# qinjr/SCoRe

Measured on AMD Instinct MI355X. Metric: train samples/sec @ batch=1024, higher is better.
Workload: dtype f32

## Files before the change

include/score_hip.h:

```cpp
#ifndef SCORE_HIP_H
#define SCORE_HIP_H

#include <stdint.h>

#ifdef __cplusplus
extern "C" {
#endif

#define SCORE_E_BADARG   (-1)
#define SCORE_E_SHAPE    (-2)
#define SCORE_E_WORKSPACE (-3)
#define SCORE_E_INDEX    (-4)

typedef void* score_context_t;
int score_context_create(score_context_t* ctx);
int score_context_destroy(score_context_t ctx);
int score_event_create(void** event);
int score_event_destroy(void* event);
int score_event_record(void* event, void* stream);
int score_stream_wait_event(void* stream, void* event);
int score_event_query(void* event);
int score_event_synchronize(void* event);

typedef struct {
// ... 178 lines not shown
  int32_t gemm_mode;
  int32_t debug_flags;
  uint8_t* row_flags;
  void* gather_done_event;
  void* plan_done_event;
  const score_step_scalars_t* step_scalars;
  score_context_t context;
  int32_t* id_status;
  void* grads_done_event;
  void* loss_done_event;
  float* loss_host;
  float* plan_workspace;
  const uint8_t* drop_mask2;
} score_state_t;

int score_id_status(int32_t* id_status, int32_t* bits, int32_t clear, void* stream);

int score_gemm_forms(const score_config_t* cfg, const score_state_t* st, int32_t B, int32_t active_slices,
                     int32_t* x_form, int32_t* dx_form);

int score_persample_form(const score_config_t* cfg, const score_state_t* st, int32_t B, int32_t active_slices);

int score_index_plan(const score_config_t* cfg, const score_state_t* st, const score_batch_t* batch,
                     int32_t n_shards, int32_t dedup, void* stream);

int score_sort_pairs(uint32_t* keys, uint32_t* vals, uint32_t* keys_alt, uint32_t* vals_alt, int64_t n, int32_t key_bits,
                     void* temp, int64_t temp_bytes, int32_t* result_in_alt, void* stream);
int64_t score_sort_pairs_temp_bytes(int64_t n);

int score_segment_sum_rows(const int32_t* rows, const float* src, int64_t n, int32_t D, int64_t n_out_rows,
                           float* out, uint8_t* row_flags, void* scratch, int64_t scratch_bytes, void* stream);
int64_t score_segment_sum_scratch_bytes(int64_t n, int32_t D);

int score_rows_accumulate(const int32_t* rows, const float* src, int64_t n, int32_t D, int64_t n_out_rows,
                          float* out, uint8_t* row_flags, void* stream);
int score_rows_accumulate_multi(const int32_t* rows, const float* src, const int64_t* offsets, int32_t n_sources, int32_t D,
                                int64_t n_out_rows, float* out, uint8_t* row_flags, void* stream);

int score_forward(const score_config_t* cfg, const score_state_t* st, const score_batch_t* batch,
                  float reg_lambda, float keep_prob, const uint8_t* drop_mask0,
                  const uint8_t* drop_mask1, uint64_t drop_seed, void* const* stage_events,
                  void* stream);

int score_backward(const score_config_t* cfg, const score_state_t* st, const score_batch_t* batch,
                   float keep_prob, float* grad_w, float* grad_table, void* const* stage_events,
                   void* stream);

typedef struct {
  const int32_t* user_seq;
  const int32_t* length;
  const int32_t* target_user;
  const int32_t* cand_items;
  const int32_t* label;
  int32_t L, C;
  int32_t active_slices;
} score_rank_batch_t;

int score_rank_workspace_bytes(const score_config_t* cfg, int32_t L, int32_t C, int64_t* bytes);
int score_rank_forward(const score_config_t* cfg, const score_state_t* st, const score_rank_batch_t* rb,
                       float reg_lambda, float* y_pred , float* loss , void* stream);

#define SCORE_CATALOG_KMAX 128
typedef struct {
  const int32_t* item_rows;
  int32_t N;
  float* zcat;
// ... 269 lines not shown
```

score_amd/_lib.py:

```python
import ctypes as C
import os

_HERE = os.path.dirname(os.path.abspath(__file__))
LIB_PATH = os.path.join(_HERE, "lib", "libscore_hip.so")

MODEL_TYPES = {"SCORE": 0, "RIA": 1, "RCA": 2, "SCORE_USER": 3, "SCORE_ITEM": 4, "RRN": 5, "GCMC": 6, "GRU4Rec": 7, "Caser": 8, "DELF": 9,
               "DEEMS": 10, "SVDpp": 11, "SASRec": 12}

MAX_PARAM_ENTRIES = 48

c_f = C.c_void_p
c_i = C.c_void_p


class Config(C.Structure):
    _fields_ = [("feature_size", C.c_int64), ("eb_dim", C.c_int32), ("hidden_size", C.c_int32),
                ("max_time_len", C.c_int32), ("obj_per_time_slice", C.c_int32),
                ("user_fnum", C.c_int32), ("item_fnum", C.c_int32), ("model_type", C.c_int32)]


class ParamEntry(C.Structure):
    _fields_ = [("name", C.c_char * 64), ("offset", C.c_int64), ("rows", C.c_int32), ("cols", C.c_int32),
                ("regularised", C.c_int32), ("init", C.c_int32)]

# ... 203 lines not shown
    "score_gemm_panel_images": [C.c_int32, C.c_int32, C.c_int32, C.c_int32, C.c_void_p, C.c_int32, c_f, C.c_int64, C.c_void_p],
    "score_gemm_panel_run": [C.c_int32, C.c_int32, C.c_int32, C.c_int32, C.c_void_p, C.c_int32, C.c_void_p, C.c_int32, C.c_void_p,
                             c_f, C.c_int64, C.c_void_p],
    "score_gemm_panel_products": [C.c_int32, C.c_int32, C.c_int32, C.c_int32, C.c_int32, C.c_void_p, C.c_int32, C.c_void_p,
                                  C.c_int32, C.c_void_p, C.c_int32, C.c_void_p, c_f, C.c_int64, C.c_void_p],
    "score_gru_fwd": [C.c_int32, C.c_int32, C.c_int32, c_f, c_f, C.c_int32, c_f, C.c_int32, c_i, c_f, C.c_int32,
                      c_f, c_f, C.c_void_p],
    "score_gru_bwd": [C.c_int32, C.c_int32, C.c_int32, c_f, C.c_int32, c_f, C.c_int32, c_i, c_f, C.c_int32, c_f,
                      c_f, C.c_int32, c_f, c_f, c_f, c_f, C.c_void_p],
    "score_adam": [c_f, c_f, c_f, c_f, C.c_int64, C.c_int64, C.c_float, C.c_float, C.c_float, C.c_float,
                   C.c_float, C.POINTER(Guard), C.c_void_p],
    "score_adam_dev": [c_f, c_f, c_f, c_f, C.c_int64, C.c_int64, C.c_float, C.c_void_p, C.c_float, C.c_float, C.c_float,
                       C.POINTER(Guard), C.c_void_p],
    "score_adam_rows_dev": [c_f, c_f, c_f, c_f, C.c_int64, C.c_int32, C.c_void_p, C.c_void_p, C.c_float, C.c_float,
                            C.c_float, C.POINTER(Guard), C.c_void_p],
    "score_adam_rows": [c_f, c_f, c_f, c_f, C.c_int64, C.c_int32, C.c_void_p, C.c_float, C.c_float, C.c_float,
                        C.c_float, C.POINTER(Guard), C.c_void_p],
    "score_adam_rows_and_dense": [c_f, c_f, c_f, c_f, C.c_int64, C.c_int32, C.c_void_p, c_f, c_f, c_f, c_f, C.c_int64, C.c_int64,
                                  C.c_float, C.c_float, C.c_float, C.c_float, C.c_float, C.POINTER(Guard), C.c_void_p],
    "score_adam_touched": [C.POINTER(AdamTable), C.c_uint32, C.c_float, C.c_void_p],
    "score_adam_touched_and_dense": [C.POINTER(AdamTable), C.c_uint32, C.c_float, c_f, c_f, c_f, c_f, C.c_int64, C.c_int64,
                                     C.c_float, C.c_void_p, C.c_void_p],
    "score_adam_unmark": [C.POINTER(AdamTable), C.c_uint32, C.c_void_p],
    "score_adam_catchup_ids": [C.POINTER(AdamTable), c_i, C.c_int64, C.c_uint32, C.c_void_p],
    "score_adam_catchup_ids_through": [C.POINTER(AdamTable), c_i, C.c_int64, C.c_uint32, C.c_float, C.c_void_p],
    "score_adam_catchup_rows": [C.POINTER(AdamTable), C.c_int64, C.c_int64, C.c_uint32, C.c_void_p],
    "score_index_plan": [C.POINTER(Config), C.POINTER(State), C.POINTER(Batch), C.c_int32, C.c_int32, C.c_void_p],
    "score_sort_pairs": [C.c_void_p, C.c_void_p, C.c_void_p, C.c_void_p, C.c_int64, C.c_int32, C.c_void_p, C.c_int64,
                         C.POINTER(C.c_int32), C.c_void_p],
    "score_sort_pairs_temp_bytes": [C.c_int64],
    "score_segment_sum_rows": [c_i, c_f, C.c_int64, C.c_int32, C.c_int64, c_f, C.c_void_p, C.c_void_p, C.c_int64,
                               C.c_void_p],
    "score_segment_sum_scratch_bytes": [C.c_int64, C.c_int32],
    "score_rows_accumulate": [c_i, c_f, C.c_int64, C.c_int32, C.c_int64, c_f, C.c_void_p, C.c_void_p],
    "score_rows_accumulate_multi": [c_i, c_f, C.POINTER(C.c_int64), C.c_int32, C.c_int32, C.c_int64, c_f, C.c_void_p, C.c_void_p],
    "score_auc_logloss": [c_f, c_i, C.c_int64, C.c_void_p, C.c_void_p, C.c_int64, C.c_void_p],
    "score_auc_scratch_bytes": [C.c_int64],
    "score_ranking_quality": [c_f, c_i, C.c_int64, C.c_int32, c_f, c_i, c_f, C.c_int64, C.c_void_p],
    "score_persample_form": [C.POINTER(Config), C.POINTER(State), C.c_int32, C.c_int32],
    "score_event_create": [C.POINTER(C.c_void_p)],
    "score_event_destroy": [C.c_void_p],
    "score_event_record": [C.c_void_p, C.c_void_p],
    "score_stream_wait_event": [C.c_void_p, C.c_void_p],
    "score_event_query": [C.c_void_p],
    "score_event_synchronize": [C.c_void_p],
    "score_abi_struct_sizes": [C.POINTER(C.c_int64), C.c_int32],
    "score_train_step": [C.POINTER(Config), C.POINTER(State), C.POINTER(Batch), C.POINTER(TrainStep), C.c_void_p],
    "score_gemm_forms": [C.POINTER(Config), C.POINTER(State), C.c_int32, C.c_int32, C.POINTER(C.c_int32), C.POINTER(C.c_int32)],
    "score_forward": [C.POINTER(Config), C.POINTER(State), C.POINTER(Batch), C.c_float, C.c_float, C.c_void_p,
                      C.c_void_p, C.c_uint64, C.POINTER(C.c_void_p), C.c_void_p],
    "score_backward": [C.POINTER(Config), C.POINTER(State), C.POINTER(Batch), C.c_float, c_f, c_f,
                       C.POINTER(C.c_void_p), C.c_void_p],
    "score_rank_workspace_bytes": [C.POINTER(Config), C.c_int32, C.c_int32, C.POINTER(C.c_int64)],
    "score_rank_forward": [C.POINTER(Config), C.POINTER(State), C.POINTER(RankBatch), C.c_float, c_f, c_f, C.c_void_p],
    "score_catalog_build": [C.POINTER(Config), C.POINTER(State), C.POINTER(Catalog), C.c_void_p],
    "score_catalog_plan": [C.POINTER(Config), C.c_int32, C.c_int32, C.c_int32, C.POINTER(C.c_int32), C.POINTER(C.c_int32),
                           C.POINTER(C.c_int64)],
    "score_catalog_topk": [C.POINTER(Config), C.POINTER(State), C.POINTER(Catalog), C.POINTER(CatalogLines), C.c_int32, c_i, c_f, c_f,
                           C.c_void_p],
    "score_catalog_struct_sizes": [C.POINTER(C.c_int64), C.c_int32],
    "score_catalog_cands_plan": [C.POINTER(Config), C.c_int32, C.c_int32, C.c_int32, C.POINTER(C.c_int32), C.POINTER(C.c_int32),
                                 C.POINTER(C.c_int64)],
    "score_catalog_topk_in": [C.POINTER(Config), C.POINTER(State), C.POINTER(Catalog), C.POINTER(CatalogLines),
                              C.POINTER(CatalogCands), C.c_int32, c_i, c_f, c_f, C.c_void_p],
    "score_catalog_cands_struct_sizes": [C.POINTER(C.c_int64), C.c_int32],
    "score_catalog_ranks_plan": [C.POINTER(Config), C.c_int32, C.c_int32, C.POINTER(C.c_int32), C.POINTER(C.c_int32),
# ... 190 lines not shown
```

score_amd/csrc/engine.hip:

```cpp
#include <string.h>
#include <stdlib.h>
#include <stdio.h>
#include <math.h>
#include <mutex>
#include <new>
#include "common.h"
#include "kernels.h"
#include "persample.h"

namespace {

const int FC1 = 200, FC2 = 80, AT1 = 80, AT2 = 40;
const int CASER_L = SCORE_CASER_L, CASER_HPAD = SCORE_CASER_HPAD;
const int MAX_ENTRIES = 48;

enum Family { FAM_SLICE, FAM_GCMC, FAM_G4R, FAM_CASER, FAM_DELF, FAM_DEEMS, FAM_SVDPP, FAM_SASREC };

struct Dims {
  int64_t N;
  int D, H, T, K, Fu, Fi, mt;
  int Du, Di, I, Dq, NI, Dk, Dhead, nstate;
  int Is[2];
  bool coattn, attn;
  Family family;
// ... 489 lines not shown
  hipStream_t st; hipEvent_t a, b, c;
  hipError_t e = hipStreamCreateWithFlags(&st, hipStreamNonBlocking);
  if (e != hipSuccess) return (int)e;
  if ((e = hipEventCreateWithFlags(&a, SCORE_DEVICE_EVENT_FLAGS)) != hipSuccess) { hipStreamDestroy(st); return (int)e; }
  if ((e = hipEventCreateWithFlags(&b, SCORE_DEVICE_EVENT_FLAGS)) != hipSuccess) { hipEventDestroy(a); hipStreamDestroy(st); return (int)e; }
  if ((e = hipEventCreateWithFlags(&c, SCORE_DEVICE_EVENT_FLAGS)) != hipSuccess) { hipEventDestroy(a); hipEventDestroy(b); hipStreamDestroy(st); return (int)e; }
  sd->st = st; sd->fork = a; sd->join = b; sd->wx = c; sd->device = dev; sd->fwd_on = nullptr;
  return 0;
}
static void side_stream_release(SideStream* sd) {
  if (!sd->st) return;
  hipStreamSynchronize(sd->st);
  hipEventDestroy(sd->fork); hipEventDestroy(sd->join); hipEventDestroy(sd->wx);
  hipStreamDestroy(sd->st);
  sd->st = nullptr;
}
#define SCORE_MAX_DEVICES 16
static SideStream g_default_ctx[SCORE_MAX_DEVICES];
static std::mutex g_default_mu;
static int side_stream(const score_state_t* st, SideStream** out) {
  if (st && st->context) { *out = reinterpret_cast<SideStream*>(st->context); return 0; }
  int dev = 0;
  if (hipGetDevice(&dev) != hipSuccess || dev < 0 || dev >= SCORE_MAX_DEVICES) return SCORE_E_BADARG;
  std::lock_guard<std::mutex> lock(g_default_mu);
  SideStream& sd = g_default_ctx[dev];
  if (!sd.st) SCORE_TRY(side_stream_create(&sd));
  *out = &sd;
  return 0;
}
enum {
  DF_GRU_STEPWISE = 1, DF_HEAD_FUSED_ANY_B = 2, DF_GRU_F32_REC = 4, DF_NO_PANEL = 8, DF_PANEL_DX = 16, DF_SORT_LIB = 32,
  DF_HEAD_UNFUSED = 64, DF_ATTN_UNFUSED = 128, DF_SORT_OWN = 256, DF_NO_PS = 512, DF_PS_FWD_ONLY = 1024, DF_PS_BWD_ONLY = 2048,
  DF_ONE_STREAM = 4096, DF_G4R_COMPOSED = 8192, DF_COATTN_ALL_ROWS = 32768,
  DF_COATTN_META_AHEAD = 65536, DF_COATTN_FWD_ONE_UNIT = 131072
};
static inline int coattn_fwd_ch_of(const score_state_t* st) { return (st->debug_flags >> 20) & 15; }
struct Flags {
  bool gru_stepwise, head_fused_any_b, gru_f32_rec, no_panel, panel_dx, sort_lib, head_unfused, attn_unfused, sort_own, no_ps,
      ps_fwd_only, ps_bwd_only, one_stream, g4r_composed, coattn_all_rows, coattn_meta_ahead, coattn_fwd_one_unit;
};
static inline Flags flags_of(const score_state_t* st) {
  auto on = [st](int bit) { return (st->debug_flags & bit) != 0; };
  Flags o;
  o.gru_stepwise = on(DF_GRU_STEPWISE); o.head_fused_any_b = on(DF_HEAD_FUSED_ANY_B); o.gru_f32_rec = on(DF_GRU_F32_REC);
  o.no_panel = on(DF_NO_PANEL); o.panel_dx = on(DF_PANEL_DX); o.sort_lib = on(DF_SORT_LIB); o.sort_own = on(DF_SORT_OWN);
  o.head_unfused = on(DF_HEAD_UNFUSED); o.attn_unfused = on(DF_ATTN_UNFUSED); o.no_ps = on(DF_NO_PS);
  o.ps_fwd_only = on(DF_PS_FWD_ONLY); o.ps_bwd_only = on(DF_PS_BWD_ONLY); o.one_stream = on(DF_ONE_STREAM);
  o.g4r_composed = on(DF_G4R_COMPOSED); o.coattn_all_rows = on(DF_COATTN_ALL_ROWS);
  o.coattn_meta_ahead = on(DF_COATTN_META_AHEAD); o.coattn_fwd_one_unit = on(DF_COATTN_FWD_ONE_UNIT);
  return o;
}
static int side_stream(const score_state_t* st, hipStream_t s, SideStream** out) {
  SideStream* real = nullptr;
  SCORE_TRY(side_stream(st, &real));
  if (!st || !flags_of(st).one_stream) { *out = real; return 0; }
  static thread_local SideStream inl;
  const hipStream_t was = inl.fwd_on;
  inl = *real; inl.st = s; inl.fwd_on = was;
  *out = &inl;
  return 0;
}
static inline int fork_side(SideStream* side, hipStream_t s) {
  HIPTRY(hipEventRecord(side->fork, s));
  HIPTRY(hipStreamWaitEvent(side->st, side->fork, 0));
  return 0;
}

#define G(call) SCORE_TRY(call)
static inline int gemm_mode_call(int x3, int tr, int M, int N, int K, const float* A, int lda, const float* B,
                                 int ldb, float* C, int ldc, const float* bias, int flags, float keep,
                                 const uint8_t* mask, uint64_t seed, float* scratch, int64_t scratch_floats,
                                 void* s) {
  return score_gemm(tr, M, N, K, A, lda, B, ldb, C, ldc, bias, flags | x3, keep, mask, seed, scratch, scratch_floats,
                    s);
}
#define EV(i) \
  do { if (stage_events && stage_events[i]) HIPTRY(hipEventRecord((hipEvent_t)stage_events[i], s)); } while (0)

static inline uint32_t clamp_rows(int64_t n) { return (uint32_t)(n < 0x80000000ll ? n : 0x80000000ll); }
static inline int global_batch(const score_state_t* st, int B) { return st->global_batch > 0 ? st->global_batch : B; }

struct Pass {
// ... 295 lines not shown
    pg.A = A ? A[side] : nullptr; pg.img = p->img[g]; pg.C = C ? C[side] + half * p->Nh : nullptr;
    pg.bias = which == 0 ? cat + (int64_t)d.Is[side] * 3 * H + half * p->Nh : nullptr;
  }
}
static int panel_prep(const Pass& c, int which, hipStream_t on) {
  PanelGroups p;
  panel_groups(c, which, nullptr, nullptr, &p);
  return score_gemm_panel_prep(p.n, p.src, 3 * c.H, p.trans, p.Nh, p.K, p.img, on);
}
static int panel_launch(const Pass& c, int which, const float* const* A, float* const* C) {
  PanelGroups p;
  panel_groups(c, which, A, C, &p);
  return score_gemm_panel(p.n, p.pg, c.BT, p.Nh, p.K, p.lda, p.ldc, c.s);
}

static int loss_tail_at(const Pass& c, SideStream* sd, float reg_lambda, int n, const float* lossb, float* loss, int Bg) {
  hipStream_t ls = c.s;
  if (c.st->loss_done_event) { G(fork_side(sd, c.s)); ls = sd->st; }
  G(score_launch_loss_final(n, lossb, loss, reg_lambda, c.ws + c.w.part, Bg, ls, c.st->id_status));
  if (c.st->loss_done_event) HIPTRY(hipEventRecord((hipEvent_t)c.st->loss_done_event, ls));
  return 0;
}
static int loss_tail(const Pass& c, SideStream* sd, float reg_lambda) {
  return loss_tail_at(c, sd, reg_lambda, c.B, c.ws + c.w.lossb, c.ws + c.w.loss, c.Bg);
}

static int row_scatter(const Pass& c, float* plan, float* grad_table) {
  const Dims& d = c.d; const Params& P = c.P; const WS& w = c.w; float* ws = c.ws; const float* W = c.W;
  PullArgs pa;
  memset(&pa, 0, sizeof(pa));
  pa.D = d.D; pa.K = d.K; pa.zero_is_dummy = 1;
  pa.flags = c.st->scatter_mode == 0 ? c.st->row_flags : nullptr;
  pa.uid = c.st->scatter_mode == 2 ? reinterpret_cast<const uint32_t*>(ws + w.uid) : nullptr;
  const float invK = 1.0f / (float)d.K;
  const float* Gm[6] = {ws + w.dxside[0], ws + w.dxside[1], ws + w.dxside[0], ws + w.dxside[1], ws + w.dtgt, ws + w.dtgt};
  const int ldg[6] = {d.I, d.I, d.I, d.I, d.Dq, d.Dq};
  const int gcol[6] = {0, d.Du, d.Di, 0, 0, d.Du};
  for (int g = 0; g < 6; ++g) { pa.G[g] = Gm[g]; pa.ldg[g] = ldg[g]; pa.gcol[g] = gcol[g]; pa.constA[g] = 1.0f; }
  if (d.coattn) {
    pa.cA[0] = ws + w.pcoef[0]; pa.cA[2] = ws + w.pcoef[1];
    pa.constA[1] = invK; pa.constA[3] = invK;
    pa.cB[0] = pa.cB[1] = ws + w.dzcoef[0]; pa.cB[2] = pa.cB[3] = ws + w.dzcoef[1];
    pa.Wv[0] = W + P.ca_w[0] + d.Di; pa.Wv[1] = W + P.ca_w[0] + 2 * d.Di;
    pa.Wv[2] = W + P.ca_w[1] + d.Du; pa.Wv[3] = W + P.ca_w[1] + 2 * d.Du;
  }
  const int64_t n_occ = (int64_t)c.B * (2 * (int64_t)c.T * d.K * (d.Fu + d.Fi) + d.Fu + d.Fi);
  return score_launch_pull(pa, reinterpret_cast<uint32_t*>(plan + w.keys_out), reinterpret_cast<uint32_t*>(plan + w.vals_out),
                           n_occ + 1, grad_table, ws + w.partials, w.partial_floats, c.s);
}

struct GradQueues { GemmQueue gq; ColsumJobs cq; };
static inline void queues_init(GradQueues* q) { q->gq.n = 0; q->cq.n = 0; q->cq.part_used = 0; }
static int queue_head(const Pass& c, GradQueues* q, float* gw, bool bn1_sums) {
  const Dims& d = c.d; const Params& P = c.P; const WS& w = c.w; float* ws = c.ws; const int B = c.B;
  G(gemm_queue_add(&q->gq, FC2, 1, B, ws + w.f2, FC2, ws + w.dlogit, 1, gw + P.fc_w[2], 1));
  G(colsum_queue_add(&q->cq, ws + w.dlogit, B, 1, 1, gw + P.fc_b[2], 0));
  G(gemm_queue_add(&q->gq, FC1, FC2, B, ws + w.f1, FC1, ws + w.dz2, FC2, gw + P.fc_w[1], FC2));
  G(colsum_queue_add(&q->cq, ws + w.dz2, B, FC2, FC2, gw + P.fc_b[1], 0));
  G(gemm_queue_add(&q->gq, d.Dhead, FC1, B, ws + w.bn, d.Dhead, ws + w.dz1, FC1, gw + P.fc_w[0], FC1));
  G(colsum_queue_add(&q->cq, ws + w.dz1, B, FC1, FC1, gw + P.fc_b[0], 0));
  if (bn1_sums) {
    G(colsum_queue_add(&q->cq, ws + w.dgstage, B, d.Dhead, d.Dhead, gw + P.bn_g, 0));
    G(colsum_queue_add(&q->cq, ws + w.dbn, B, d.Dhead, d.Dhead, gw + P.bn_b, 0));
  }
  return 0;
}
// ... 1546 lines not shown
```

score_amd/csrc/kernels.h:

```cpp
#pragma once
#include "common.h"

#define GEMM_GROUP_MAX 16
struct GemmProb {
  const float* A; const float* B; float* C; float* slab;
  const float* bias;
  int M, N, K, lda, ldb, ldc, k_chunk, gx, gy, nblocks;
};
struct GemmGroup { int n; int total_blocks; GemmProb p[GEMM_GROUP_MAX]; };
enum { GF_BIAS = 1, GF_RELU = 2, GF_ACC = 4, GF_DROP = 8, GF_X3 = 16, GF_X3F = 32, GF_RELUGRAD = 64 };
__device__ __forceinline__ int64_t bias_index(int flags, int row, int col, int N) {
  const int g = flags >> 16;
  return g ? (int64_t)(row / g) * N + col : col;
}
__device__ __forceinline__ float gemm_epilogue(float v, int row, int col, int N, const float* bias, int flags,
                                               float keep, const uint8_t* mask, uint64_t seed) {
  if (flags & GF_BIAS) v += bias[bias_index(flags, row, col, N)];
  if (flags & GF_RELU) v = fmaxf(v, 0.f);
  if (flags & GF_DROP) {
    uint64_t e = (uint64_t)row * (uint64_t)N + (uint64_t)col;
    bool on = mask ? (mask[e] != 0) : (hash_uniform(seed, e) < keep);
    v = on ? v / keep : 0.f;
  }
  if (flags & GF_RELUGRAD) {
// ... 112 lines not shown
                                float* logit, float* y, float* lossb, float* dlogit, int Bglobal, hipStream_t s,
                                const uint64_t* seed_dev = nullptr, float* dz2 = nullptr, int single_launch = 0);
bool score_head_fwd_fused_fits(int B, int Dh, int N1, int N2);
int score_launch_head_bwd_fused(int B, int Dh, int N1, int N2, const float* dz2, const float* W2, const float* f1, float keep,
                                const float* W1, const float* x, const float* gamma, float rs, float* dz1, float* dbn,
                                float* dhead, float* tmp, hipStream_t s);
int score_launch_attn_fwd_fused(int B, int T, int H, int NI, int N1, int N2, const float* q, const float* ur,
                                const float* ir, const float* info, const float* Weff, const float* qz, const float* W4,
                                const float* b4, const float* w5, const float* b5, const int32_t* length, float* inp,
                                float* a1, float* a2, float* score, float* head, int ldh, int off_u, int off_i,
                                hipStream_t s, int weff_copies = 1, int64_t weff_copy_stride = 0);
int score_launch_outer_relu_bwd(int B, int NF, const float* dlogit, const float* w, const float* f, float keep,
                                float* dz, hipStream_t s);
int score_launch_copy2d(int64_t rows, int cols, const float* src, int lds_, float* dst, int ldd, hipStream_t s);

struct PlanFillArgs {
  const int32_t* idx[6];
  int64_t off[7];
  int F[6];
  int K, G, shift;
  int T, TA;
  uint32_t n_rows;
  int32_t* id_status;
};
struct PullArgs {
  const float* G[6]; int ldg[6]; int gcol[6];
  const float* cA[6]; const float* cB[6];
  const float* Wv[6];
  float constA[6];
  const uint32_t* uid;
  int D, K, LPRp;
  int zero_is_dummy;
  uint8_t* flags;
};
struct PlanRemapArgs { int32_t* out[6]; int F[6]; int K; int T, TA; };
int score_launch_plan_unique(const PlanRemapArgs& ra, const uint32_t* keys, const uint32_t* vals, int64_t n,
                             uint32_t* flags_scratch, uint32_t* uid, uint32_t* unique_keys, int32_t* unique_rows,
                             int32_t* meta, int G, int shift, void* temp, size_t temp_bytes, hipStream_t s);
int score_scan_temp_bytes(int64_t n, size_t* bytes);
int score_plan_temp_bytes(int64_t n, int end_bit, size_t* bytes);
int score_launch_plan(const PlanFillArgs& a, int key_bits, uint32_t* keys_in, uint32_t* vals_in, uint32_t* keys_out,
                      uint32_t* vals_out, void* temp, size_t temp_bytes, hipStream_t s, int which = 0);
int score_launch_plan_own(const PlanFillArgs& a, int key_bits, uint32_t* keys_in, uint32_t* vals_in, uint32_t* keys_out,
                          uint32_t* vals_out, void* temp, size_t temp_bytes, hipStream_t s);
size_t score_sort_temp_bytes(int64_t n);
int score_pull_window(int64_t n);
int score_launch_pull(PullArgs& a, const uint32_t* keys, const uint32_t* vals, int64_t n, float* out,
                      float* partials, int64_t partial_floats, hipStream_t s);

struct GruSide {
  const float* xproj;
  const float* Wg; int ldwg;
  const float* Wc; int ldwc;
  float* out; int ldo;
  float* gates;
  float* final_state;
  const float* dout; int lddo;
  const float* dfinal;
  float* dxproj;
  float* rh;
  float* hprev;
  float* bias_slab;
  const int32_t* length;
};
struct GruArgs {
  GruSide s[2];
// ... 155 lines not shown
```

score_amd/csrc/scatter.hip:

```cpp
#include <cstring>
#include <cstdlib>
#include <rocprim/device/device_radix_sort.hpp>
#include <rocprim/device/device_scan.hpp>
#include "common.h"
#include "kernels.h"

#define DESC(seg, f, k, bt) (((uint32_t)(seg) << 29) | ((uint32_t)(f) << 26) | ((uint32_t)(k) << 21) | (uint32_t)(bt))

__global__ void plan_fill_kernel(PlanFillArgs a, uint32_t* __restrict__ keys, uint32_t* __restrict__ vals) {
  int64_t i = (int64_t)blockIdx.x * blockDim.x + threadIdx.x;
  if (i > a.off[6]) return;
  if (i == a.off[6]) {
    keys[i] = 0;
    vals[i] = DESC(7, 0, 0, 0);
    return;
  }
  int seg = 0;
#pragma unroll
  for (int s = 1; s < 6; ++s) seg += (i >= a.off[s]) ? 1 : 0;
  int64_t local = i - a.off[seg];
  const uint32_t F = (uint32_t)a.F[seg];
  uint32_t f, k, bt;
  const uint32_t l32 = (uint32_t)local;
  if (seg < 4) {
    const uint32_t q = l32 / F;
    f = l32 - q * F;
    bt = q / (uint32_t)a.K;
    k = q - bt * (uint32_t)a.K;
    if (a.TA != a.T) {
      const uint32_t b = bt / (uint32_t)a.TA;
      local = (((int64_t)b * a.T + (bt - b * (uint32_t)a.TA)) * a.K + k) * F + f;
    }
  } else {
    bt = l32 / F;
// ... 215 lines not shown
      vv[u] = vals[idx];
    }
    if (has_uid) {
#pragma unroll
      for (int u = 0; u < PULL_U; ++u) uu[u] = a.uid[i0 + u < end ? i0 + u : end - 1];
    } else {
#pragma unroll
      for (int u = 0; u < PULL_U; ++u) uu[u] = kk[u];
    }
#pragma unroll
    for (int u = 0; u < PULL_U; ++u) cc[u] = pull_contrib_t<MODE>(a, tab, vv[u], ch4);
#pragma unroll
    for (int u = 0; u < PULL_U; ++u) {
      if (i0 + u >= end) break;
      const uint32_t key = kk[u];
      if (key != cur) {
        if (cur != 0 || !a.zero_is_dummy) {
          if (is_first && first_open) st4(pfirst + w * a.D + ch4, acc);
          else store_cur();
        }
        acc = make_float4(0.f, 0.f, 0.f, 0.f);
        cur = key;
        cur_dst = uu[u];
        is_first = false;
      }
      if (key != 0 || !a.zero_is_dummy) acc = add4(acc, cc[u]);
    }
  }
  if (cur != 0 || !a.zero_is_dummy) {
    const bool open_right = end < n && keys[end] == cur;
    if (is_first && first_open) st4(pfirst + w * a.D + ch4, acc);
    else if (open_right) st4(plast + w * a.D + ch4, acc);
    else store_cur();
  }
}

__device__ __forceinline__ int64_t run_end(const uint32_t* __restrict__ keys, int64_t lo, int64_t n, uint32_t key) {
  int64_t step = 1, hi = n;
  while (lo + step < n) {
    if (keys[lo + step - 1] != key) { hi = lo + step - 1; break; }
    lo += step;
    step <<= 1;
  }
  while (lo < hi) {
    int64_t mid = (lo + hi) >> 1;
    if (keys[mid] == key) lo = mid + 1; else hi = mid;
  }
  return lo;
}

#define LONG_CHAIN 16
__global__ __launch_bounds__(256) void pull_fixup_kernel(const PullArgs a, const uint32_t* __restrict__ keys,
                                                         int64_t n, int WS, float* __restrict__ out,
                                                         const float* __restrict__ pfirst,
                                                         const float* __restrict__ plast) {
  extern __shared__ float sh[];
  __shared__ int2 s_long[256];
  __shared__ int s_nlong;
  const int LPR = a.LPRp;
  const int gpb = blockDim.x / LPR;
  const int g = threadIdx.x / LPR;
  const int64_t w = (int64_t)blockIdx.x * gpb + g;
  const int ch4 = (threadIdx.x % LPR) * 4;
  const bool lane_ok = ch4 < a.D;
  if (threadIdx.x == 0) s_nlong = 0;
  __syncthreads();
// ... 23 lines not shown
    const int L = e.y;
    const int chunk = (L + gpb - 1) / gpb;
    const int j0 = 1 + g * chunk, j1 = min(L, (g + 1) * chunk);
    float4 tot = make_float4(0.f, 0.f, 0.f, 0.f);
    if (lane_ok) {
      float4 t8[8];
#pragma unroll
      for (int q = 0; q < 8; ++q) t8[q] = make_float4(0.f, 0.f, 0.f, 0.f);
      int j = j0;
      for (; j + 7 <= j1; j += 8) {
        float4 v[8];
#pragma unroll
        for (int q = 0; q < 8; ++q) v[q] = ld4(pfirst + (wl + j + q) * a.D + ch4);
#pragma unroll
        for (int q = 0; q < 8; ++q) t8[q] = add4(t8[q], v[q]);
      }
      for (; j <= j1; ++j) t8[0] = add4(t8[0], ld4(pfirst + (wl + j) * a.D + ch4));
      tot = add4(add4(add4(t8[0], t8[1]), add4(t8[2], t8[3])), add4(add4(t8[4], t8[5]), add4(t8[6], t8[7])));
      st4(sh + g * a.D + ch4, tot);
    }
    __syncthreads();
    if (g == 0 && lane_ok) {
      float4 t = ld4(plast + wl * a.D + ch4);
      for (int q = 0; q < gpb; ++q) t = add4(t, ld4(sh + q * a.D + ch4));
      const uint32_t key = keys[(wl + 1) * (int64_t)WS - 1];
      store_row(a, out, key, (wl + 1) * (int64_t)WS - 1, ch4, t);
    }
    __syncthreads();
  }
}

int score_pull_window(int64_t n) { return n >= (1 << 20) ? 64 : n >= (1 << 19) ? 32 : n >= (1 << 18) ? 16 : 8; }

int score_launch_pull(PullArgs& a, const uint32_t* keys, const uint32_t* vals, int64_t n, float* out,
                      float* partials, int64_t partial_floats, hipStream_t s) {
  const int WS = score_pull_window(n);
  int LPR = 1;
  while (LPR < a.D / 4) LPR <<= 1;
  if (LPR > 64) return SCORE_E_SHAPE;
  a.LPRp = LPR;
  int64_t nw = cdiv64(n, WS);
  if (2 * nw * a.D > partial_floats) return SCORE_E_WORKSPACE;
  float* pfirst = partials;
  float* plast = partials + nw * a.D;
  int gpb = 256 / LPR;
  unsigned blocks = (unsigned)cdiv64(nw, gpb);
  const int mode = (a.G[1] == nullptr && a.ldg[0] == 0) ? 0 : (a.cA[0] ? 2 : 1);
  if (mode == 0) hipLaunchKernelGGL(pull_kernel<0>, dim3(blocks), dim3(256), 0, s, a, keys, vals, n, WS, out, pfirst, plast);
  else if (mode == 1) hipLaunchKernelGGL(pull_kernel<1>, dim3(blocks), dim3(256), 0, s, a, keys, vals, n, WS, out, pfirst, plast);
  else hipLaunchKernelGGL(pull_kernel<2>, dim3(blocks), dim3(256), 0, s, a, keys, vals, n, WS, out, pfirst, plast);
  SCORE_CHECK_LAUNCH();
  hipLaunchKernelGGL(pull_fixup_kernel, dim3(blocks), dim3(256), (size_t)gpb * a.D * sizeof(float), s, a, keys, n, WS, out,
                     pfirst, plast);
  SCORE_CHECK_LAUNCH();
  return 0;
}

int score_rowsum_temp_bytes(int64_t n, size_t* bytes) { return score_plan_temp_bytes(n, 32, bytes); }

extern "C" int score_segment_sum_rows(const int32_t* rows, const float* src, int64_t n, int32_t D, int64_t n_out_rows,
                                      float* out, uint8_t* row_flags, void* scratch, int64_t scratch_bytes,
                                      void* stream) {
  if (!rows || !src || !out || !scratch || n < 0 || D <= 0 || (D & 3) || n_out_rows <= 0) return SCORE_E_BADARG;
  if (n == 0) return 0;
  if (n >= (1 << 29)) return SCORE_E_SHAPE;
  hipStream_t s = (hipStream_t)stream;
  size_t sort_bytes = 0;
  SCORE_TRY(score_plan_temp_bytes(n, 32, &sort_bytes));
  const int64_t nw = cdiv64(n, score_pull_window(n));
  const int64_t partial_floats = 2 * nw * D + 8 + 2 * nw;
  const int64_t need = 4 * align_up64(n, 4) * 4 + align_up64(partial_floats, 4) * 4 + (int64_t)sort_bytes;
  if (need > scratch_bytes) return SCORE_E_WORKSPACE;
  uint32_t* keys_in = static_cast<uint32_t*>(scratch);
  uint32_t* keys_out = keys_in + align_up64(n, 4);
  uint32_t* vals_in = keys_out + align_up64(n, 4);
  uint32_t* vals_out = vals_in + align_up64(n, 4);
  float* partials = reinterpret_cast<float*>(vals_out + align_up64(n, 4));
  void* temp = partials + align_up64(partial_floats, 4);
  hipLaunchKernelGGL(rowsum_fill_kernel, dim3((unsigned)cdiv64(n, 256)), dim3(256), 0, s, rows, n, keys_in, vals_in);
  SCORE_CHECK_LAUNCH();
  int key_bits = 1;
// ... 188 lines not shown
```

Measured before the change: 961,100.

## Add lane-parallel pull kernel with DPP broadcasts for model-segment embedding gradients

Adds a new pull kernel variant that loads a group's keys and descriptors cooperatively across lanes, then uses DPP broadcasts to share them. It precomputes a per-segment offset table relative to a single 32-bit base so that gradient gathers use 32-bit offsets. This replaces per-lane serial descriptor decoding and 64-bit address math in the segment-sum gather. The kernel is used when the span fits in 4 GiB and D is 16, 32 or 64, with a debug flag to fall back to the old kernel. The cost is a more complex kernel, which risks register pressure and correctness problems at segment boundaries.

```diff
diff --git a/include/score_hip.h b/include/score_hip.h
--- a/include/score_hip.h
+++ b/include/score_hip.h
@@ -234,6 +234,9 @@
                            float* out, uint8_t* row_flags, void* scratch, int64_t scratch_bytes, void* stream);
 int64_t score_segment_sum_scratch_bytes(int64_t n, int32_t D);
 
+int score_pull_form(int32_t D, int32_t mode, int64_t span_bytes);
+int score_pull_last_form(void);
+
 int score_rows_accumulate(const int32_t* rows, const float* src, int64_t n, int32_t D, int64_t n_out_rows,
                           float* out, uint8_t* row_flags, void* stream);
 int score_rows_accumulate_multi(const int32_t* rows, const float* src, const int64_t* offsets, int32_t n_sources, int32_t D,
diff --git a/score_amd/_lib.py b/score_amd/_lib.py
--- a/score_amd/_lib.py
+++ b/score_amd/_lib.py
@@ -259,6 +259,8 @@
     "score_segment_sum_rows": [c_i, c_f, C.c_int64, C.c_int32, C.c_int64, c_f, C.c_void_p, C.c_void_p, C.c_int64,
                                C.c_void_p],
     "score_segment_sum_scratch_bytes": [C.c_int64, C.c_int32],
+    "score_pull_form": [C.c_int32, C.c_int32, C.c_int64],
+    "score_pull_last_form": [],
     "score_rows_accumulate": [c_i, c_f, C.c_int64, C.c_int32, C.c_int64, c_f, C.c_void_p, C.c_void_p],
     "score_rows_accumulate_multi": [c_i, c_f, C.POINTER(C.c_int64), C.c_int32, C.c_int32, C.c_int64, c_f, C.c_void_p, C.c_void_p],
     "score_auc_logloss": [c_f, c_i, C.c_int64, C.c_void_p, C.c_void_p, C.c_int64, C.c_void_p],
diff --git a/score_amd/csrc/engine.hip b/score_amd/csrc/engine.hip
--- a/score_amd/csrc/engine.hip
+++ b/score_amd/csrc/engine.hip
@@ -545,12 +545,12 @@
   DF_GRU_STEPWISE = 1, DF_HEAD_FUSED_ANY_B = 2, DF_GRU_F32_REC = 4, DF_NO_PANEL = 8, DF_PANEL_DX = 16, DF_SORT_LIB = 32,
   DF_HEAD_UNFUSED = 64, DF_ATTN_UNFUSED = 128, DF_SORT_OWN = 256, DF_NO_PS = 512, DF_PS_FWD_ONLY = 1024, DF_PS_BWD_ONLY = 2048,
   DF_ONE_STREAM = 4096, DF_G4R_COMPOSED = 8192, DF_COATTN_ALL_ROWS = 32768,
-  DF_COATTN_META_AHEAD = 65536, DF_COATTN_FWD_ONE_UNIT = 131072
+  DF_COATTN_META_AHEAD = 65536, DF_COATTN_FWD_ONE_UNIT = 131072, DF_PULL_OLD_FORM = 262144
 };
 static inline int coattn_fwd_ch_of(const score_state_t* st) { return (st->debug_flags >> 20) & 15; }
 struct Flags {
   bool gru_stepwise, head_fused_any_b, gru_f32_rec, no_panel, panel_dx, sort_lib, head_unfused, attn_unfused, sort_own, no_ps,
-      ps_fwd_only, ps_bwd_only, one_stream, g4r_composed, coattn_all_rows, coattn_meta_ahead, coattn_fwd_one_unit;
+      ps_fwd_only, ps_bwd_only, one_stream, g4r_composed, coattn_all_rows, coattn_meta_ahead, coattn_fwd_one_unit, pull_old_form;
 };
 static inline Flags flags_of(const score_state_t* st) {
   auto on = [st](int bit) { return (st->debug_flags & bit) != 0; };
@@ -561,6 +561,7 @@
   o.ps_fwd_only = on(DF_PS_FWD_ONLY); o.ps_bwd_only = on(DF_PS_BWD_ONLY); o.one_stream = on(DF_ONE_STREAM);
   o.g4r_composed = on(DF_G4R_COMPOSED); o.coattn_all_rows = on(DF_COATTN_ALL_ROWS);
   o.coattn_meta_ahead = on(DF_COATTN_META_AHEAD); o.coattn_fwd_one_unit = on(DF_COATTN_FWD_ONE_UNIT);
+  o.pull_old_form = on(DF_PULL_OLD_FORM);
   return o;
 }
 static int side_stream(const score_state_t* st, hipStream_t s, SideStream** out) {
@@ -922,6 +923,9 @@
   pa.D = d.D; pa.K = d.K; pa.zero_is_dummy = 1;
   pa.flags = c.st->scatter_mode == 0 ? c.st->row_flags : nullptr;
   pa.uid = c.st->scatter_mode == 2 ? reinterpret_cast<const uint32_t*>(ws + w.uid) : nullptr;
+  pa.force_old = c.fl.pull_old_form ? 1 : 0;
+  const int nf[6] = {d.Fi, d.Fi, d.Fu, d.Fu, d.Fu, d.Fi};
+  for (int g = 0; g < 6; ++g) { pa.nf[g] = nf[g]; pa.rows[g] = g < 4 ? (int64_t)c.B * c.T : (int64_t)c.B; }
   const float invK = 1.0f / (float)d.K;
   const float* Gm[6] = {ws + w.dxside[0], ws + w.dxside[1], ws + w.dxside[0], ws + w.dxside[1], ws + w.dtgt, ws + w.dtgt};
   const int ldg[6] = {d.I, d.I, d.I, d.I, d.Dq, d.Dq};
diff --git a/score_amd/csrc/kernels.h b/score_amd/csrc/kernels.h
--- a/score_amd/csrc/kernels.h
+++ b/score_amd/csrc/kernels.h
@@ -168,6 +168,8 @@
   int D, K, LPRp;
   int zero_is_dummy;
   uint8_t* flags;
+  int nf[6]; int64_t rows[6];
+  int force_old;
 };
 struct PlanRemapArgs { int32_t* out[6]; int F[6]; int K; int T, TA; };
 int score_launch_plan_unique(const PlanRemapArgs& ra, const uint32_t* keys, const uint32_t* vals, int64_t n,
diff --git a/score_amd/csrc/scatter.hip b/score_amd/csrc/scatter.hip
--- a/score_amd/csrc/scatter.hip
+++ b/score_amd/csrc/scatter.hip
@@ -1,5 +1,6 @@
 #include <cstring>
 #include <cstdlib>
+#include <type_traits>
 #include <rocprim/device/device_radix_sort.hpp>
 #include <rocprim/device/device_scan.hpp>
 #include "common.h"
@@ -281,6 +282,199 @@
     if (is_first && first_open) st4(pfirst + w * a.D + ch4, acc);
     else if (open_right) st4(plast + w * a.D + ch4, acc);
     else store_cur();
+  }
+}
+
+struct PullLaneSeg { uint32_t goff, ldg4, caoff, cboff; float constA; int useA; };
+struct PullLanes {
+  const char* base;
+  PullLaneSeg seg[6];
+  const float* Wv[6];
+  int nf[6];
+};
+typedef __attribute__((address_space(1))) char gchar;
+typedef __attribute__((address_space(1))) score_v4f gv4f;
+
+template <int LPR, int U>
+__device__ __forceinline__ int grp_bcast_c(int v) {
+  if (LPR == 16) return __builtin_amdgcn_update_dpp(0, v, 0x150 + U, 0xf, 0xf, true);
+  if (LPR == 8) {
+    const int r = __builtin_amdgcn_update_dpp(0, v, 0x150 + (U & 7), 0xf, 0x3, false);
+    return __builtin_amdgcn_update_dpp(r, v, 0x150 + (U & 7) + 8, 0xf, 0xc, false);
+  }
+  return __builtin_amdgcn_update_dpp(0, v, (U & 3) * 0x55, 0xf, 0xf, true);
+}
+template <int LPR>
+__device__ __forceinline__ int grp_bcast(int v, int u) {
+  switch (u) {
+    case 0: return grp_bcast_c<LPR, 0>(v);   case 1: return grp_bcast_c<LPR, 1>(v);
+    case 2: return grp_bcast_c<LPR, 2>(v);   case 3: return grp_bcast_c<LPR, 3>(v);
+    case 4: return grp_bcast_c<LPR, 4>(v);   case 5: return grp_bcast_c<LPR, 5>(v);
+    case 6: return grp_bcast_c<LPR, 6>(v);   case 7: return grp_bcast_c<LPR, 7>(v);
+    case 8: return grp_bcast_c<LPR, 8>(v);   case 9: return grp_bcast_c<LPR, 9>(v);
+    case 10: return grp_bcast_c<LPR, 10>(v); case 11: return grp_bcast_c<LPR, 11>(v);
+    case 12: return grp_bcast_c<LPR, 12>(v); case 13: return grp_bcast_c<LPR, 13>(v);
+    case 14: return grp_bcast_c<LPR, 14>(v); default: return grp_bcast_c<LPR, 15>(v);
+  }
+}
+
+template <int MODE, int LPR, int TU>
+__global__ __launch_bounds__(256) void pull_kernel_lanes(const PullArgs a, const PullLanes la,
+                                                         const uint32_t* __restrict__ keys,
+                                                         const uint32_t* __restrict__ vals, int64_t n, int WS,
+                                                         float* __restrict__ out, float* __restrict__ pfirst,
+                                                         float* __restrict__ plast) {
+#pragma clang fp contract(off)
+  static_assert(MODE == 1 || MODE == 2, "model segments only");
+  static_assert((LPR == 4 || LPR == 8 || LPR == 16) && (TU == 8 || TU == 16), "a group inside one DPP row");
+  constexpr int D = LPR * 4, GPB = 256 / LPR;
+  constexpr int NM = TU > LPR ? TU / LPR : 1;
+  const int j = threadIdx.x % LPR;
+  const int64_t w = (int64_t)blockIdx.x * GPB + threadIdx.x / LPR;
+  __shared__ PullLaneSeg tab[6];
+  __shared__ float4 wvs[MODE == 2 ? 6 * 8 * LPR : 1];
+  if (threadIdx.x == 0) {
+#pragma unroll
+    for (int sg = 0; sg < 6; ++sg) tab[sg] = la.seg[sg];
+  }
+  if (MODE == 2) {
+    float4 t[6];
+#pragma unroll
+    for (int sg = 0; sg < 6; ++sg)
+      t[sg] = ld4_global(la.Wv[sg] + ((int)threadIdx.x < la.nf[sg] * LPR ? threadIdx.x * 4 : 0));
+#pragma unroll
+    for (int sg = 0; sg < 6; ++sg)
+      if ((int)threadIdx.x < la.nf[sg] * LPR) wvs[sg * 8 * LPR + threadIdx.x] = t[sg];
+  }
+  __syncthreads();
+  const int64_t start = w * WS;
+  if (start >= n) return;
+  const int64_t end = start + WS < n ? start + WS : n;
+  const int len = (int)(end - start);
+  const uint32_t* __restrict__ kp = keys + start;
+  const uint32_t* __restrict__ vp = vals + start;
+  const uint32_t* __restrict__ dp = a.uid ? a.uid + start : kp;
+  uint32_t lastk = kp[len - 1], leftk = keys[start > 0 ? start - 1 : 0];
+  uint32_t cur = kp[0], cur_dst = dp[0];
+  uint32_t key[NM], desc[NM], dstv[NM];
+#pragma unroll
+  for (int r = 0; r < NM; ++r) {
+    const int pos = r * LPR + j < len - 1 ? r * LPR + j : len - 1;
+    key[r] = kp[pos]; desc[r] = vp[pos]; dstv[r] = dp[pos];
+  }
+  asm volatile("" : "+v"(leftk), "+v"(cur), "+v"(cur_dst));
+#pragma unroll
+  for (int r = 0; r < NM; ++r) asm volatile("" : "+v"(key[r]), "+v"(desc[r]), "+v"(dstv[r]));
+  if (a.zero_is_dummy && lastk == 0) return;
+  const bool first_open = start > 0 && leftk == cur;
+  const bool dummy = a.zero_is_dummy != 0;
+  bool is_first = true;
+  float4 acc = make_float4(0.f, 0.f, 0.f, 0.f);
+  const gchar* base = (const gchar*)la.base;
+  const int gsh = (threadIdx.x & 63) & ~(LPR - 1);
+  auto store_out = [&](uint32_t dst) {
+    st4(out + (int64_t)dst * D + j * 4, acc);
+    if (a.flags && j == 0) a.flags[dst] = 2;
+  };
+  for (int t0 = 0; t0 < len; t0 += TU) {
+    uint32_t goff[NM];
+    int wvi[NM];
+    float ca[NM], cb[NM], pa[NM], pb[NM];
+    int useA[NM];
+#pragma unroll
+    for (int r = 0; r < NM; ++r) {
+      int seg = desc[r] >> 29;
+      seg = seg > 5 ? 5 : seg;
+      const uint32_t f = (desc[r] >> 26) & 7, k = (desc[r] >> 21) & 31, bt = desc[r] & 0x1FFFFF;
+      const PullLaneSeg si = tab[seg];
+      goff[r] = si.goff + bt * si.ldg4 + f * (D * 4);
+      wvi[r] = seg * 8 * LPR + (int)f * LPR;
+      ca[r] = si.constA; cb[r] = 0.f; useA[r] = si.useA; pa[r] = 0.f; pb[r] = 0.f;
+      if (MODE == 2) {
+        const uint32_t co = (bt * (uint32_t)a.K + k) * 4;
+        pa[r] = *(const gfloat*)(base + (uint64_t)(si.caoff + co));
+        pb[r] = *(const gfloat*)(base + (uint64_t)(si.cboff + co));
+      }
+    }
+    score_v4f g[TU];
+#pragma unroll
+    for (int u = 0; u < TU; ++u) {
+      const uint32_t o = (uint32_t)grp_bcast<LPR>((int)goff[u / LPR], u % LPR) + j * 16;
+      g[u] = *(const gv4f*)(base + (uint64_t)o);
+    }
+    uint32_t nkey[NM], ndesc[NM], ndst[NM];
+#pragma unroll
+    for (int r = 0; r < NM; ++r) {
+      const int pos = t0 + TU + r * LPR + j < len - 1 ? t0 + TU + r * LPR + j : len - 1;
+      nkey[r] = kp[pos]; ndesc[r] = vp[pos]; ndst[r] = dp[pos];
+    }
+    const int cnt = len - t0;
+    uint32_t prevk[NM], prevd[NM], gm = 0;
+    bool head[NM];
+#pragma unroll
+    for (int r = 0; r < NM; ++r) {
+      const bool valid = r * LPR + j < TU && r * LPR + j < cnt;
+      const uint32_t ck = r == 0 ? cur : (uint32_t)grp_bcast<LPR>((int)key[r > 0 ? r - 1 : 0], LPR - 1);
+      const uint32_t cd = r == 0 ? cur_dst : (uint32_t)grp_bcast<LPR>((int)dstv[r > 0 ? r - 1 : 0], LPR - 1);
+      prevk[r] = (uint32_t)__builtin_amdgcn_update_dpp((int)ck, (int)key[r], 0x111, 0xf, 0xf, false);
+      prevd[r] = (uint32_t)__builtin_amdgcn_update_dpp((int)cd, (int)dstv[r], 0x111, 0xf, 0xf, false);
+      prevk[r] = j == 0 ? ck : prevk[r];
+      prevd[r] = j == 0 ? cd : prevd[r];
+      head[r] = valid && key[r] != prevk[r];
+      gm |= ((uint32_t)(__ballot(head[r]) >> gsh) & ((1u << (TU < LPR ? TU : LPR)) - 1u)) << (r * LPR);
+    }
+    int meta[NM];
+#pragma unroll
+    for (int r = 0; r < NM; ++r) {
+      const bool valid = r * LPR + j < TU && r * LPR + j < cnt;
+      int act = 0;
+      if (head[r])
+        act = (prevk[r] == 0 && dummy) ? 3 : ((is_first && first_open && (gm & ((1u << (r * LPR + j)) - 1u)) == 0) ? 2 : 1);
+      meta[r] = act | (valid ? 4 : 0) | (wvi[r] << 3);
+      if (MODE == 2) {
+        ca[r] = (useA[r] & 1) ? pa[r] : ca[r];
+        cb[r] = (useA[r] & 2) ? pb[r] : 0.f;
+      }
+    }
+    is_first = is_first && gm == 0;
+    cur = (uint32_t)grp_bcast<LPR>((int)key[NM - 1], (TU - 1) % LPR);
+    cur_dst = (uint32_t)grp_bcast<LPR>((int)dstv[NM - 1], (TU - 1) % LPR);
+    auto consume = [&](auto chk) {
+      constexpr bool CHECK = decltype(chk)::value;
+      int m = grp_bcast<LPR>(meta[0], 0);
+      float4 wv = make_float4(0.f, 0.f, 0.f, 0.f), wv_n = wv;
+      if (MODE == 2) wv = wvs[(m >> 3) + j];
+#pragma unroll
+      for (int u = 0; u < TU; ++u) {
+        const int m_n = u + 1 < TU ? grp_bcast<LPR>(meta[(u + 1 < TU ? u + 1 : u) / LPR], (u + 1) % LPR) : 0;
+        if (MODE == 2 && u + 1 < TU) wv_n = wvs[(m_n >> 3) + j];
+        const uint32_t d_u = (uint32_t)grp_bcast<LPR>((int)prevd[u / LPR], u % LPR);
+        const float ca_u = __int_as_float(grp_bcast<LPR>(__float_as_int(ca[u / LPR]), u % LPR));
+        if (m & 3) {
+          if ((m & 3) == 1) store_out(d_u);
+          else if ((m & 3) == 2) st4(pfirst + w * D + j * 4, acc);
+          acc = make_float4(0.f, 0.f, 0.f, 0.f);
+        }
+        float4 r;
+        r.x = ca_u * g[u].x; r.y = ca_u * g[u].y; r.z = ca_u * g[u].z; r.w = ca_u * g[u].w;
+        if (MODE == 2) {
+          const float cb_u = __int_as_float(grp_bcast<LPR>(__float_as_int(cb[u / LPR]), u % LPR));
+          r = fma4(cb_u, wv, r);
+        }
+        if (!CHECK || (m & 4)) { acc.x = acc.x + r.x; acc.y = acc.y + r.y; acc.z = acc.z + r.z; acc.w = acc.w + r.w; }
+        m = m_n; wv = wv_n;
+      }
+    };
+    if (cnt >= TU) consume(std::false_type());
+    else consume(std::true_type());
+#pragma unroll
+    for (int r = 0; r < NM; ++r) { key[r] = nkey[r]; desc[r] = ndesc[r]; dstv[r] = ndst[r]; }
+  }
+  if (cur != 0 || !dummy) {
+    const bool open_right = end < n && keys[end] == cur;
+    if (is_first && first_open) st4(pfirst + w * D + j * 4, acc);
+    else if (open_right) st4(plast + w * D + j * 4, acc);
+    else store_out(cur_dst);
   }
 }
 
@@ -370,6 +564,62 @@
 
 int score_pull_window(int64_t n) { return n >= (1 << 20) ? 64 : n >= (1 << 19) ? 32 : n >= (1 << 18) ? 16 : 8; }
 
+extern "C" int score_pull_form(int32_t D, int32_t mode, int64_t span_bytes) {
+  if (mode != 1 && mode != 2) return 0;
+  if (D != 16 && D != 32 && D != 64) return 0;
+  return span_bytes > 0 && span_bytes <= ((int64_t)1 << 32) ? 1 : 0;
+}
+static int g_pull_last_form = -1;
+extern "C" int score_pull_last_form(void) { return g_pull_last_form; }
+
+static bool pull_lanes_table(const PullArgs& a, int mode, PullLanes* L, int64_t* span) {
+  const char* lo = nullptr; const char* hi = nullptr;
+  const float* Ge[6]; const float* cAe[6]; const float* cBe[6];
+  for (int sg = 0; sg < 6; ++sg) {
+    if (a.nf[sg] <= 0 || a.nf[sg] > 8 || a.rows[sg] <= 0 || a.rows[sg] > (1 << 21)) return false;
+    const int c = sg < 4 ? ((sg & 2) ? 2 : 0) : 0;
+    Ge[sg] = a.G[sg] ? a.G[sg] : a.G[4];
+    cAe[sg] = a.cA[c]; cBe[sg] = a.cB[c];
+    L->Wv[sg] = a.Wv[sg < 4 ? sg : sg - 4];
+    L->nf[sg] = a.nf[sg];
+    if (!Ge[sg] || a.ldg[sg] < 0 || a.gcol[sg] < 0) return false;
+    if (mode == 2 && (!cAe[sg] || !cBe[sg] || !L->Wv[sg])) return false;
+  }
+  auto reach = [&](const float* p, int64_t floats) {
+    const char* b = reinterpret_cast<const char*>(p);
+    if (!lo || b < lo) lo = b;
+    if (!hi || b + floats * 4 > hi) hi = b + floats * 4;
+  };
+  for (int sg = 0; sg < 6; ++sg) {
+    reach(Ge[sg], (a.rows[sg] - 1) * a.ldg[sg] + a.gcol[sg] + (int64_t)a.nf[sg] * a.D);
+    if (mode == 2) { reach(cAe[sg], a.rows[sg] * a.K); reach(cBe[sg], a.rows[sg] * a.K); }
+  }
+  *span = hi - lo;
+  if (*span > ((int64_t)1 << 32)) return false;
+  L->base = lo;
+  for (int sg = 0; sg < 6; ++sg) {
+    PullLaneSeg& t = L->seg[sg];
+    t.goff = (uint32_t)(reinterpret_cast<const char*>(Ge[sg]) - lo) + (uint32_t)a.gcol[sg] * 4u;
+    t.ldg4 = (uint32_t)a.ldg[sg] * 4u;
+    t.caoff = mode == 2 ? (uint32_t)(reinterpret_cast<const char*>(cAe[sg]) - lo) : 0u;
+    t.cboff = mode == 2 ? (uint32_t)(reinterpret_cast<const char*>(cBe[sg]) - lo) : 0u;
+    t.constA = a.constA[sg];
+    t.useA = (sg < 4 && a.cA[sg] ? 1 : 0) | (sg < 4 && a.cB[sg] ? 2 : 0);
+  }
+  return true;
+}
+
+template <int MODE>
+static void pull_lanes_launch(const PullArgs& a, const PullLanes& L, int LPR, int WS, unsigned blocks, const uint32_t* keys,
+                              const uint32_t* vals, int64_t n, float* out, float* pfirst, float* plast, hipStream_t s) {
+#define PULL_LANES_GO(lpr, tu) \
+  hipLaunchKernelGGL((pull_kernel_lanes<MODE, lpr, tu>), dim3(blocks), dim3(256), 0, s, a, L, keys, vals, n, WS, out, pfirst, plast)
+  if (LPR == 4) PULL_LANES_GO(4, 8);
+  else if (LPR == 8) { if (WS < 16) PULL_LANES_GO(8, 8); else PULL_LANES_GO(8, 16); }
+  else { if (WS < 16) PULL_LANES_GO(16, 8); else PULL_LANES_GO(16, 16); }
+#undef PULL_LANES_GO
+}
+
 int score_launch_pull(PullArgs& a, const uint32_t* keys, const uint32_t* vals, int64_t n, float* out,
                       float* partials, int64_t partial_floats, hipStream_t s) {
   const int WS = score_pull_window(n);
@@ -384,7 +634,15 @@
   int gpb = 256 / LPR;
   unsigned blocks = (unsigned)cdiv64(nw, gpb);
   const int mode = (a.G[1] == nullptr && a.ldg[0] == 0) ? 0 : (a.cA[0] ? 2 : 1);
-  if (mode == 0) hipLaunchKernelGGL(pull_kernel<0>, dim3(blocks), dim3(256), 0, s, a, keys, vals, n, WS, out, pfirst, plast);
+  PullLanes L;
+  int64_t span = 0;
+  const bool lanes = !a.force_old && mode != 0 && pull_lanes_table(a, mode, &L, &span) && score_pull_form(a.D, mode, span);
+  g_pull_last_form = lanes ? 1 : 0;
+  if (lanes) {
+    if (mode == 1) pull_lanes_launch<1>(a, L, LPR, WS, blocks, keys, vals, n, out, pfirst, plast, s);
+    else pull_lanes_launch<2>(a, L, LPR, WS, blocks, keys, vals, n, out, pfirst, plast, s);
+  }
+  else if (mode == 0) hipLaunchKernelGGL(pull_kernel<0>, dim3(blocks), dim3(256), 0, s, a, keys, vals, n, WS, out, pfirst, plast);
   else if (mode == 1) hipLaunchKernelGGL(pull_kernel<1>, dim3(blocks), dim3(256), 0, s, a, keys, vals, n, WS, out, pfirst, plast);
   else hipLaunchKernelGGL(pull_kernel<2>, dim3(blocks), dim3(256), 0, s, a, keys, vals, n, WS, out, pfirst, plast);
   SCORE_CHECK_LAUNCH();
```

New measurement: 976,900 (median of 6 runs). 1.02x the previous value.
